# dannyfa/VAE-GAM

Hardware: AMD Instinct MI355X
Metric: fMRI volumes/sec/train-step (41x49x35) (higher is better)
Workload: dtype f32; 1 GPU; configs[2] full VAE-GAM: B=64/GPU C=8, 41x49x35, 2 subj x 98 vol synthetic checker, fwd+bwd+Adam, hipGraph replay; global_batch=64, covariates=8, parallelism=dp1

## Files before the change

include/vaegam.h:

```cpp
#ifndef VAEGAM_H
#define VAEGAM_H
#include <stdint.h>
#ifdef __cplusplus
extern "C" {
#endif

typedef struct vg_conv_desc {
    int32_t N;
    int32_t CI, CO;
    int32_t ID, IH, IW;
    int32_t OD, OH, OW;
    int32_t KD, KH, KW;
    int32_t stride;
    int32_t pad_d, pad_h, pad_w;
    int32_t relu_in;
    int32_t per_group;
    int32_t relu_out;
} vg_conv_desc;

int         vg_version(void);
const char* vg_last_error(void);

int vg_corr3d(const vg_conv_desc* d, const float* x, const float* wpk, const float* bias,
              const float* in_scale, const float* in_shift, const float* mask_src, float* y, void* stream);

int vg_tconv3d_s2(const vg_conv_desc* d, const float* x, const float* wpk, const float* bias,
                  const float* in_scale, const float* in_shift, const float* mask_src, float* y, void* stream);
int64_t vg_tconv3d_s2_stats_chunks(const vg_conv_desc* d, int32_t stats_per_group);
int vg_tconv3d_s2_stats(const vg_conv_desc* d, const float* x, const float* wpk, const float* bias,
                        const float* in_scale, const float* in_shift, float* y, int32_t stats_per_group,
                        int32_t stats_relu, double* stats_part, void* stream);

#define VG_CONV_PLAN_LEN 36
int vg_corr3d_plan(const vg_conv_desc* d, int32_t has_prologue, int32_t* out, int32_t n_out);
int vg_tconv3d_s2_plan(const vg_conv_desc* d, int32_t has_prologue, int32_t stats_per_group, int32_t* out, int32_t n_out);

typedef struct vg_mm_desc {
    int32_t N, CI, CO;
    int32_t ID, IH, IW, OD, OH, OW;
    int32_t nq, ks[4];
    int32_t PDT, PH, PW, PD;
    int32_t sdi, shi, swi, d0, LD, cc;
    int32_t sdo, sho, swo, od0[4], oh0[4], ow0[4];
    int32_t relu_in, per_group, tpc, slack;
    int32_t dbuf;
    int32_t PHB;
    int32_t hlo, hhi;
    int32_t waves;
    int32_t relu_out;
} vg_mm_desc;
int64_t vg_conv_mm_stats_chunks(const vg_mm_desc* d, int32_t stats_per_group);
int vg_conv_mm(const vg_mm_desc* d, const float* x, const float* a_img, const int32_t* tau, const int32_t* dlt, const float* bias,
               const float* in_scale, const float* in_shift, const float* mask_src, float* y, int32_t stats_per_group,
               int32_t stats_relu, double* stats_part, void* stream);
int vg_gather_f32(const float* src, const int32_t* idx, float* dst, int64_t n, void* stream);

typedef struct vg_wgrad_desc {
    int32_t N, CB, CA;
    int32_t PD, PH, PW;
    int32_t AD, AH, AW;
    int32_t KD, KH, KW;
    int32_t stride;
    int32_t pad_d, pad_h, pad_w;
    int32_t pro_on_a;
// ... 179 lines not shown
```

vae-gam_amd/_lib.py:

```python
import ctypes
import os

import torch

_HERE = os.path.dirname(os.path.abspath(__file__))
LIB_NAME = 'libvaegam_hip.so'

i32, i64, f32, f64, vp = ctypes.c_int32, ctypes.c_int64, ctypes.c_float, ctypes.c_double, ctypes.c_void_p


class ConvDesc(ctypes.Structure):
    _fields_ = [(n, i32) for n in ('N', 'CI', 'CO', 'ID', 'IH', 'IW', 'OD', 'OH', 'OW', 'KD', 'KH', 'KW',
                                   'stride', 'pad_d', 'pad_h', 'pad_w', 'relu_in', 'per_group', 'relu_out')]


class WgradDesc(ctypes.Structure):
    _fields_ = [(n, i32) for n in ('N', 'CB', 'CA', 'PD', 'PH', 'PW', 'AD', 'AH', 'AW', 'KD', 'KH', 'KW',
                                   'stride', 'pad_d', 'pad_h', 'pad_w', 'pro_on_a', 'relu_in', 'per_group')]


class MmDesc(ctypes.Structure):
    _fields_ = [(n, i32) for n in ('N', 'CI', 'CO', 'ID', 'IH', 'IW', 'OD', 'OH', 'OW', 'nq')] + [('ks', i32 * 4)] + \
               [(n, i32) for n in ('PDT', 'PH', 'PW', 'PD', 'sdi', 'shi', 'swi', 'd0', 'LD', 'cc', 'sdo', 'sho', 'swo')] + \
               [('od0', i32 * 4), ('oh0', i32 * 4), ('ow0', i32 * 4)] + [(n, i32) for n in ('relu_in', 'per_group', 'tpc', 'slack', 'dbuf', 'PHB', 'hlo', 'hhi', 'waves',
                                                                                         'relu_out')]


class GainDesc(ctypes.Structure):
    _fields_ = [('C', i32), ('B', i32), ('n', i32), ('hrf_taps', i32), ('jitter_b', f64), ('jitter_ku', f64), ('prior_var', f64)]


class FcDesc(ctypes.Structure):
    _fields_ = [('M', i32), ('N', i32), ('K', i32), ('batch', i32), ('a_sm', i64), ('a_sk', i64), ('a_sb', i64),
                ('b_sk', i64), ('b_sn', i64), ('b_sb', i64), ('c_sm', i64), ('c_sb', i64), ('bias_sb', i64), ('cx_sb', i64),
                ('ksplit', i32), ('flags', i32)]


class FcJob(ctypes.Structure):
    _fields_ = [('d', FcDesc), ('A', vp), ('amask', vp), ('B', vp), ('bias', vp), ('cmask', vp), ('C', vp), ('cx', vp), ('ws', vp)]

# ... 1 lines not shown
class VolFile(ctypes.Structure):
    _fields_ = [('offset', i64), ('sx', i64), ('sy', i64), ('sz', i64), ('st', i64), ('slope', f64), ('inter', f64),
                ('dtype', i32), ('swap', i32), ('scale', i32), ('reserved', i32)]


FC_A_RELU, FC_A_MASK, FC_B_RELU, FC_B_ONES, FC_C_BIAS, FC_C_RELU, FC_C_MASK, FC_C_ACCUM = 1, 2, 4, 8, 16, 32, 64, 128


_PROTOS = {
    'vg_version': (ctypes.c_int, []),
    'vg_last_error': (ctypes.c_char_p, []),
    'vg_corr3d': (ctypes.c_int, [ctypes.POINTER(ConvDesc), vp, vp, vp, vp, vp, vp, vp, vp]),
    'vg_tconv3d_s2': (ctypes.c_int, [ctypes.POINTER(ConvDesc), vp, vp, vp, vp, vp, vp, vp, vp]),
    'vg_tconv3d_s2_stats_chunks': (i64, [ctypes.POINTER(ConvDesc), i32]),
    'vg_tconv3d_s2_stats': (ctypes.c_int, [ctypes.POINTER(ConvDesc), vp, vp, vp, vp, vp, vp, i32, i32, vp, vp]),
    'vg_corr3d_plan': (ctypes.c_int, [ctypes.POINTER(ConvDesc), i32, ctypes.POINTER(i32), i32]),
    'vg_tconv3d_s2_plan': (ctypes.c_int, [ctypes.POINTER(ConvDesc), i32, i32, ctypes.POINTER(i32), i32]),
    'vg_bn_stats_from_parts': (ctypes.c_int, [vp, i32, i32, i64, f64, vp, vp, f32, vp, vp, vp, vp, vp, vp, vp]),
    'vg_wgrad3d_ws_bytes': (i64, [ctypes.POINTER(WgradDesc)]),
    'vg_wgrad3d': (ctypes.c_int, [ctypes.POINTER(WgradDesc), vp, vp, vp, vp, vp, vp, i32, vp]),
    'vg_wgrad3d_grouped_ws_bytes': (i64, [ctypes.POINTER(WgradDesc)]),
    'vg_wgrad3d_grouped': (ctypes.c_int, [ctypes.POINTER(WgradDesc), vp, vp, vp, vp, vp, vp, vp]),
    'vg_wgrad3d_plan': (ctypes.c_int, [ctypes.POINTER(WgradDesc), i32, ctypes.POINTER(i32), i32]),
    'vg_bn_tconv1_sums': (ctypes.c_int, [vp, vp, vp, vp, i32, i32, i32, vp, vp, i32, vp]),
    'vg_bn_ws_bytes': (i64, [i32, i32, i64, i32]),
    'vg_bn_plan': (ctypes.c_int, [i32, i32, i64, i32, ctypes.POINTER(i32)]),
    'vg_bn_stats': (ctypes.c_int, [vp, i32, i32, i64, i32, i32, vp, vp, f32, vp, vp, vp, vp, vp, vp, vp]),
    'vg_bn_finalize': (ctypes.c_int, [vp, i32, i32, vp, vp, f32, vp, vp, vp, vp, vp]),
    'vg_bn_bwd_reduce': (ctypes.c_int, [vp, vp, i32, i32, i64, i32, i32, vp, vp, vp, vp, vp]),
    'vg_bn_bwd_apply': (ctypes.c_int, [vp, vp, i32, i32, i64, i32, i32, vp, vp, vp, vp, f64, vp, vp, vp, vp, i32, vp]),
# ... 105 lines not shown
```

vae-gam_amd/csrc/vg_conv.hip:

```cpp
#include "vg_common.h"
#include <stdlib.h>
#include "../../include/vaegam.h"

namespace {

struct CorrParams {
    vg_conv_desc d;
    int TWG, TH, TD;
    int tilesW, tilesH, tilesD;
};

__device__ __forceinline__ int clampi(int v, int lo, int hi) { return min(max(v, lo), hi); }

struct ConvQuery { int32_t* plan; int64_t* chunks; int small; };
enum { FAM_DIRECT = 0, FAM_PLANE = 1, FAM_TCONV = 2 };

template <int COT, int KD, int KH, int KW, int S, int TDt, int THt, int TW, int COC>
__global__ void __launch_bounds__(256)
corr3d_direct_k(const float* __restrict__ x, const float* __restrict__ wpk, const float* __restrict__ bias,
         const float* __restrict__ in_scale, const float* __restrict__ in_shift,
         const float* __restrict__ mask_src, float* __restrict__ y, CorrParams p) {
    constexpr int KVOL = KD * KH * KW;
    constexpr int RW = (TW - 1) * S + KW;
    constexpr int RD = (TDt - 1) * S + KD;
// ... 637 lines not shown
        const size_t chunks = (size_t)stats_pg * gridDim.x * nw;
        const size_t chunk = ((size_t)(n % stats_pg) * gridDim.x + blockIdx.x) * nw + wv;
#pragma unroll
        for (int co = 0; co < COT; ++co) {
            float a = st_s[co], b = st_q[co];
#pragma unroll
            for (int off = 32; off > 0; off >>= 1) { a += __shfl_xor(a, off); b += __shfl_xor(b, off); }
            if (lane == 0) {
                double* dst = stats_part + (((size_t)g * CO + co0 + co) * chunks + chunk) * 2;
                dst[0] = (double)a; dst[1] = (double)b;
            }
        }
    }
}

template <int COT, int KD, int KH, int KW, int COC = 0>
int launch_tconv(const vg_conv_desc* d, const float* x, const float* wpk, const float* bias, const float* in_scale,
                 const float* in_shift, const float* mask_src, float* y, hipStream_t s,
                 double* stats_part = nullptr, int stats_relu = 0, int stats_pg = 1, const ConvQuery* query = nullptr) {
    TconvParams p; p.d = *d;
    p.JD = (d->OD + d->pad_d + 1) / 2; p.JH = (d->OH + d->pad_h + 1) / 2; p.JW = (d->OW + d->pad_w + 1) / 2;
    p.TJW = p.JW < 32 ? p.JW : 32;
    int rem = 256 / p.TJW;
    p.TJH = p.JH < rem ? p.JH : rem;
    rem = 256 / (p.TJW * p.TJH);
    p.TJD = p.JD < rem ? p.JD : rem;
    if (p.TJD < 1) p.TJD = 1;
    p.tilesW = vg_cdiv(p.JW, p.TJW); p.tilesH = vg_cdiv(p.JH, p.TJH); p.tilesD = vg_cdiv(p.JD, p.TJD);
    if (d->CO % COT) { vg_set_error("tconv3d_s2: CO=%d not a multiple of %d", d->CO, COT); return VG_ERR_UNSUPPORTED; }
    const int threads = vg_cdiv(p.TJW * p.TJH * p.TJD, VG_WAVE) * VG_WAVE;
    dim3 grid(p.tilesW * p.tilesH * p.tilesD, d->N, d->CO / COT);
    const bool nopro = in_scale == nullptr && !d->relu_in;
    if (query) {
        const int64_t chunks = (int64_t)stats_pg * grid.x * (threads / VG_WAVE);
        if (query->chunks) *query->chunks = chunks;
        if (query->plan) {
            const int32_t rec[VG_CONV_PLAN_LEN] = {
                FAM_TCONV, COT, KD, KH, KW, 2, 2, 2, 2, COC, nopro ? 1 : 0, query->small, p.TJW, p.TJH, p.TJD, p.tilesW, p.tilesH, p.tilesD,
                threads, (int32_t)grid.x, (int32_t)grid.y, (int32_t)grid.z, 0, 0, 0, 0, 0, 0, 0, 0, 0, 0, p.JD, p.JH, p.JW, (int32_t)chunks};
            for (int i = 0; i < VG_CONV_PLAN_LEN; ++i) query->plan[i] = rec[i];
        }
        return VG_OK;
    }
    if (nopro)
        vg_launch(tconv3d_s2_k<COT, KD, KH, KW, COC, true>, grid, dim3(threads), 0, s,
// ... 139 lines not shown
    ConvQuery q = {out, nullptr, 0};
    rc = tconv_dispatch(d, &dummy, &dummy, nullptr, pro, pro, nullptr, &dummy, nullptr, nullptr, 0, stats_per_group > 0 ? stats_per_group : 1, &q);
    if (rc == VG_OK && stats_per_group <= 0) out[VG_CONV_PLAN_LEN - 1] = 0;
    return rc;
}

extern "C" int vg_tconv3d_s2_stats(const vg_conv_desc* d, const float* x, const float* wpk, const float* bias,
                                   const float* in_scale, const float* in_shift, float* y, int32_t stats_per_group,
                                   int32_t stats_relu, double* stats_part, void* stream) {
    int rc = tconv_check(d, x, wpk, in_scale, in_shift, y);
    if (rc) return rc;
    if (!stats_part || stats_per_group <= 0 || d->N % stats_per_group) { vg_set_error("vg_tconv3d_s2_stats: bad statistics arguments"); return VG_ERR_ARG; }
    return tconv_dispatch(d, x, wpk, bias, in_scale, in_shift, nullptr, y, (hipStream_t)stream, stats_part, stats_relu,
                          stats_per_group, nullptr);
}
```

vae-gam_amd/csrc/vg_conv_mm.hip:

```cpp
#include "vg_common.h"
#include <stdlib.h>
#include <stdint.h>
#include <type_traits>
#include "../../include/vaegam.h"

#ifdef VG_STAMP
__device__ unsigned long long vg_stamp_out[1024 * 16 * 8];
#define VG_STAMP_T(t) do { __builtin_amdgcn_sched_barrier(0); asm volatile("s_memtime %0\n\ts_waitcnt lgkmcnt(0)" : "=s"(t) :: "memory"); __builtin_amdgcn_sched_barrier(0); } while (0)
#define VG_STAMP_ADD(i) do { unsigned long long t_; VG_STAMP_T(t_); st_sum[i] += t_ - st_last; st_last = t_; } while (0)
#else
#define VG_STAMP_ADD(i) do {} while (0)
#endif

namespace {

constexpr int MM_MAXQ = 4;
constexpr int MM_ZPAD = 64;

struct MmParams {
    vg_mm_desc d;
    int bps, nsplit;
    int ksbase[MM_MAXQ], a_off[MM_MAXQ];
    int kstot, aimg_floats;
    int a_res;
    int CHP, buf_floats;
    int nhb, PHB, h0, LH, LPH;
    int tau_off, in_off;
    int has_pro;
};

struct alignas(16) mm_f4 { float v[4]; };

template <int V> struct mm_int { static constexpr int value = V; };
template <int MAXN, typename F>
__device__ __forceinline__ void mm_dispatch(int n, F&& f) {
    if constexpr (MAXN >= 1) {
// ... 8 lines not shown

template <int MM_W, int NQ, int TPC, int K0, int K1, int K2, int K3, bool DB, int OCC, bool MASKED>
__global__ void __launch_bounds__(MM_W * VG_WAVE, OCC)
conv_mm_k(const float* __restrict__ x, const float* __restrict__ a_img, const int* __restrict__ tau, const int* __restrict__ dlt,
          const float* __restrict__ bias, const float* __restrict__ in_scale, const float* __restrict__ in_shift,
          const float* __restrict__ mask_src, float* __restrict__ y, double* __restrict__ stats_part, int stats_pg, int stats_relu,
          MmParams p) {
    VG_DYN_SMEM(float, lds);
    constexpr int MM_T = MM_W * VG_WAVE;
    const vg_mm_desc& d = p.d;
    float* Al = lds;
    int* Tl = reinterpret_cast<int*>(lds + p.tau_off);
    float* In = lds + p.in_off;
    const int tid = threadIdx.x, lane = tid % VG_WAVE, wave = vg_wave_id();
    const int kk = lane >> 4, jl = lane & 15;
    const int b = blockIdx.x % p.bps, split = blockIdx.x / p.bps;
    const int IHW = d.IH * d.IW, OHW = d.OH * d.OW;
    const int CI = d.CI, CO = d.CO;
    constexpr bool STATIC_K = K0 > 0;
    constexpr int KSUM = K0 + K1 + K2 + K3;

    for (int i = tid; i < p.aimg_floats; i += MM_T) Al[i] = a_img[i];
    if (!STATIC_K) for (int i = tid; i < p.kstot * 64; i += MM_T) {
        const int* e = dlt + ((i >> 6) * 4 + ((i & 63) >> 4)) * 3;
        Tl[i] = e[0] * p.LPH + e[1] * d.IW + e[2];
    }
    for (int i = tid; i < (DB ? 2 : 1) * d.cc * MM_ZPAD; i += MM_T) In[(i / MM_ZPAD) * p.CHP + (i % MM_ZPAD)] = 0.f;

    const int bd = b / p.nhb, bh = b - bd * p.nhb;
    const int pd0 = bd * d.PD, ph0 = bh * p.PHB;
    const int npd = min(d.PD, d.PDT - pd0), nph = min(p.PHB, d.PH - ph0);
// ... 56 lines not shown
            }
        }
    }
    const float lo = d.relu_in ? 0.f : -__builtin_inff();
    const int nchunks = (CI + d.cc - 1) / d.cc;
    const int nsamp = (d.N - split + p.nsplit - 1) / p.nsplit;
    const int units = nsamp * nchunks;

    vg_f32x4 acc[TPC];
#pragma unroll
    for (int i = 0; i < TPC; ++i) { acc[i].v[0] = 0.f; acc[i].v[1] = 0.f; acc[i].v[2] = 0.f; acc[i].v[3] = 0.f; }
    vg_f2 st_s[2] = {{0.f, 0.f}, {0.f, 0.f}}, st_q[2] = {{0.f, 0.f}, {0.f, 0.f}};
    float mreg[MASKED ? TPC : 1][4];
    vg_f2 bias_l[2];
#pragma unroll
    for (int r = 0; r < 2; ++r) { bias_l[r].x = bias ? bias[co_l + 2 * r] : 0.f; bias_l[r].y = bias ? bias[co_l + 2 * r + 1] : 0.f; }
    int nact = 0;
#pragma unroll
    for (int i = 0; i < TPC; ++i) nact += (i * MM_W + wave < ntiles) ? 1 : 0;

    int nst[NQ];
#pragma unroll
    for (int q = 0; q < NQ; ++q) {
        int c4 = 0;
#pragma unroll
        for (int i = 0; i < TPC; ++i) c4 += (vg_any(((vbits >> (q * TPC + i)) & 1u) != 0) && i < nact) ? 4 : 0;
        nst[q] = c4;
    }

    auto load_mask = [&](int n) __attribute__((always_inline)) {
        const char* mn = reinterpret_cast<const char*>(mask_src + (size_t)n * CO * ovol);
#pragma unroll
        for (int i = 0; i < TPC; ++i) {
            const bool okt = i < nact && ((vbits >> i) & 1u);
            const unsigned off = okt ? ob[i] + 4u * (unsigned)(d.od0[0] * OHW + d.oh0[0] * d.OW + d.ow0[0]) : 0u;
#pragma unroll
            for (int r = 0; r < 4; ++r)
                mreg[i][r] = okt ? *reinterpret_cast<const float*>(mn + (size_t)r * ovol * 4 + off) : 0.f;
        }
    };
    auto store_class_t = [&](int n, int q, auto relu_c, auto stats_c, auto srelu_c) __attribute__((always_inline)) {
        constexpr bool RELU = !MASKED && decltype(relu_c)::value;
        constexpr bool STATS = decltype(stats_c)::value, SRELU = decltype(srelu_c)::value;
        const long long cq4 = 4ll * (d.od0[q] * OHW + d.oh0[q] * d.OW + d.ow0[q]);
        const size_t ovol4 = ovol * 4;
        char* yq = reinterpret_cast<char*>(y + (size_t)n * CO * ovol) + cq4;
        const char* mq = reinterpret_cast<const char*>(mask_src + (size_t)n * CO * ovol) + cq4;
        float* yr[4]; const float* mr[4];
#pragma unroll
        for (int r = 0; r < 4; ++r) { yr[r] = reinterpret_cast<float*>(yq + r * ovol4); mr[r] = reinterpret_cast<const float*>(mq + r * ovol4); }
        vg_touch(vbits);
#pragma unroll
        for (int i = 0; i < TPC; ++i) {
            if ((vbits >> (q * TPC + i)) & 1u) {
                vg_touch(ob[i]);
                const unsigned off = ob[i];
                float mk[4];
                if constexpr (MASKED) {
#pragma unroll
                    for (int r = 0; r < 4; ++r) {
                        if constexpr (NQ == 1) mk[r] = mreg[i][r];
                        else mk[r] = vg_load_sbase(mr[r], off);
// ... 48 lines not shown
            else if (emode == 4) store_class_t(n, q, F{}, T{}, T{});
            else store_class_t(n, q, T{}, T{}, F{});
        }
    };
    auto flush_stats = [&](int n) __attribute__((always_inline)) {
        const int g = n / stats_pg;
        const size_t chunks = (size_t)stats_pg * p.bps * MM_W;
        const size_t chunkid = ((size_t)(n % stats_pg) * p.bps + b) * MM_W + wave;
#pragma unroll
        for (int r = 0; r < 4; ++r) {
            float sa = (r & 1) ? st_s[r >> 1].y : st_s[r >> 1].x, sb = (r & 1) ? st_q[r >> 1].y : st_q[r >> 1].x;
#pragma unroll
            for (int off = 8; off > 0; off >>= 1) { sa += __shfl_xor(sa, off); sb += __shfl_xor(sb, off); }
            if (CO == 8) { sa += __shfl_xor(sa, 32); sb += __shfl_xor(sb, 32); }
            if (jl == 0 && (CO == 16 || kk < 2)) {
                double* dst = stats_part + (((size_t)g * CO + co_l + r) * chunks + chunkid) * 2;
                dst[0] = (double)sa; dst[1] = (double)sb;
            }
        }
#pragma unroll
        for (int r = 0; r < 2; ++r) { st_s[r].x = 0.f; st_s[r].y = 0.f; st_q[r].x = 0.f; st_q[r].y = 0.f; }
    };

    const int nsp = d.cc * nspan_c;
    const int parts = (nsp >= MM_W) ? 1 : (MM_W + nsp - 1) / nsp;
    const int head = dst0 & 3;
    const int n4 = (head + span_fl + 3) >> 2;
    const int n4p = (n4 + parts - 1) / parts;
    auto stage = [&](int u) __attribute__((always_inline)) {
        const int n = split + (u / nchunks) * p.nsplit, c0 = (u % nchunks) * d.cc;
        const int cc = min(d.cc, CI - c0);
// ... 157 lines not shown

}

#ifdef VG_STAMP
extern "C" int vg_stamp_read(unsigned long long* dst, int n) {
    return (int)hipMemcpyFromSymbol(dst, HIP_SYMBOL(vg_stamp_out), sizeof(unsigned long long) * n, 0, hipMemcpyDeviceToHost);
}
#endif

static int mm_plan_params(const vg_mm_desc* d, MmParams* p, size_t* shmem, const char* who) {
    if (!d || d->N <= 0 || d->CI <= 0 || (d->CO != 8 && d->CO != 16) || d->nq < 1 || d->nq > MM_MAXQ || d->PD <= 0 || d->PDT <= 0 ||
        d->PH <= 0 || d->PW <= 0 || d->slack < 0 || d->PH > 1023 || d->PW > 1023 || d->PD > 1023 || d->cc <= 0 || d->LD <= 0 || d->tpc <= 0) {
        vg_set_error("%s: bad descriptor", who); return VG_ERR_ARG;
    }
    p->d = *d;
    int row = 0, af = 0;
    for (int q = 0; q < d->nq; ++q) {
        if (d->ks[q] <= 0 || d->ks[q] > 32) { vg_set_error("%s: k-steps per channel must be 1..32 (class %d: %d)", who, q, d->ks[q]); return VG_ERR_ARG; }
        p->ksbase[q] = row; p->a_off[q] = af;
        row += d->ks[q]; af += d->CI * d->ks[q] * 64;
    }
    p->kstot = row; p->aimg_floats = af;
    if (d->nq > 1 && d->cc < d->CI) { vg_set_error("%s: multi-class plans need all input channels in one chunk", who); return VG_ERR_ARG; }
    const int IHW = d->IH * d->IW;
    const int W = d->waves;
    if (W != 4 && W != 8) { vg_set_error("%s: waves per workgroup must be 4 or 8 (got %d)", who, W); return VG_ERR_ARG; }
    if (d->hhi < d->hlo) { vg_set_error("%s: bad row-offset range [%d, %d]", who, d->hlo, d->hhi); return VG_ERR_ARG; }
    p->PHB = (d->PHB > 0 && d->PHB < d->PH) ? d->PHB : d->PH;
    p->nhb = vg_cdiv(d->PH, p->PHB);
    p->h0 = d->hlo;
// ... 22 lines not shown

extern "C" int vg_conv_mm(const vg_mm_desc* d, const float* x, const float* a_img, const int32_t* tau, const int32_t* dlt,
                          const float* bias, const float* in_scale, const float* in_shift, const float* mask_src, float* y,
                          int32_t stats_per_group, int32_t stats_relu, double* stats_part, void* stream) {
    MmParams p{}; size_t shmem;
    int rc = mm_plan_params(d, &p, &shmem, "vg_conv_mm");
    if (rc) return rc;
    if (!x || !a_img || !tau || !dlt || !y) { vg_set_error("vg_conv_mm: null argument"); return VG_ERR_ARG; }
    if ((in_scale == nullptr) != (in_shift == nullptr) || (in_scale && d->per_group <= 0)) { vg_set_error("vg_conv_mm: in_scale/in_shift/per_group inconsistent"); return VG_ERR_ARG; }
    if (stats_part && (stats_per_group <= 0 || d->N % stats_per_group)) { vg_set_error("vg_conv_mm: bad statistics arguments"); return VG_ERR_ARG; }
    p.has_pro = (d->relu_in || in_scale) ? 1 : 0;
    hipStream_t s = (hipStream_t)stream;
    const int threads = d->waves * VG_WAVE;
    auto launch = [&](auto kernel) {
        const int bpc = vg_blocks_per_cu((const void*)kernel, threads, shmem);
        int ns = (256 * bpc) / p.bps; if (ns < 1) ns = 1; if (ns > d->N) ns = d->N;
        p.nsplit = ns;
        vg_launch(kernel, dim3(p.bps * p.nsplit), dim3(threads), shmem, s, x, a_img, (const int*)tau, (const int*)dlt, bias, in_scale, in_shift,
                  mask_src, y, stats_part, (int)(stats_part ? stats_per_group : 1), (int)stats_relu, p);
    };
    const bool db = d->dbuf != 0, mk = mask_src != nullptr, w4 = d->waves == 4;
#define MM_LAUNCH_W(W, NQ, TPC, K0, K1, K2, K3) { \
        constexpr int OCC_ = (TPC * (K0 + K1 + K2 + K3) + 10 * TPC <= 96 && K0 > 0) ? 4 : 2; \
        if (db) { if (mk) launch(conv_mm_k<W, NQ, TPC, K0, K1, K2, K3, true, OCC_, true>); else launch(conv_mm_k<W, NQ, TPC, K0, K1, K2, K3, true, OCC_, false>); } \
        else    { if (mk) launch(conv_mm_k<W, NQ, TPC, K0, K1, K2, K3, false, OCC_, true>); else launch(conv_mm_k<W, NQ, TPC, K0, K1, K2, K3, false, OCC_, false>); } }
#define MM_LAUNCH(NQ, TPC, K0, K1, K2, K3) { if (w4) MM_LAUNCH_W(4, NQ, TPC, K0, K1, K2, K3) else MM_LAUNCH_W(8, NQ, TPC, K0, K1, K2, K3) }
#define MM_TPC(NQ, K0, K1, K2, K3) \
    { if (d->tpc <= 3) MM_LAUNCH(NQ, 3, K0, K1, K2, K3) else if (d->tpc <= 4) MM_LAUNCH(NQ, 4, K0, K1, K2, K3) else if (d->tpc <= 5) MM_LAUNCH(NQ, 5, K0, K1, K2, K3) \
      else if (d->tpc <= 6) MM_LAUNCH(NQ, 6, K0, K1, K2, K3) else MM_LAUNCH(NQ, 8, K0, K1, K2, K3) }
    const int* k = d->ks;
    if (d->nq == 1 && d->tpc <= 8) {
        if (k[0] == 7) MM_TPC(1, 7, 0, 0, 0)
        else if (k[0] == 9) MM_TPC(1, 9, 0, 0, 0)
// ... 32 lines not shown
```

vae-gam_amd/ops.py:

```python
import ctypes
from collections import namedtuple
from dataclasses import dataclass
from typing import Optional, Tuple

import torch

from . import _lib
from ._lib import ConvDesc, WgradDesc

BN_EPS = 1e-5

PROFILE = None
_LABEL = ['']


class label:
    def __init__(self, name):
        self.name = name

    def __enter__(self):
        self.prev = _LABEL[0]; _LABEL[0] = self.name

    def __exit__(self, *a):
        _LABEL[0] = self.prev
# ... 462 lines not shown
    def forward(ctx, p_in, weight, bias, gamma, beta, spec: ConvSpec, relu_in: bool, per_group: int,
                input_is_data: bool, sync, packed=None, next_bn=None, pre_stats=None, producer_bias=None,
                bias_grad_by_consumer=False, relu_out=False, rectified_in=False):
        p_in = p_in.contiguous()
        has_bn = gamma is not None
        assert not rectified_in or relu_in, 'rectified_in: p_in = relu(p) only stands in for p where the layer rectifies its input'
        fwd_relu = relu_in and not (rectified_in and not has_bn)
        assert producer_bias is None or has_bn, 'producer_bias: the hand-off happens in the batch-norm backward'
        scale = shift = mean = rstd = None
        part = None
        with label(spec.name + '/fwd'):
            if has_bn:
                scale, shift, mean, rstd = bn_stats(p_in, gamma, beta, relu_in, per_group, sync, pre_stats)
            mmf = _mm_for(packed, weight, spec, 'fwd', tuple(p_in.shape[2:]), None)
            if mmf is not None:
                y = conv_mm(p_in, mmf[0], mmf[1], bias, fwd_relu, scale, shift, per_group, None, next_bn, relu_out)
            else:
                wf = packed.get(spec.name, 'fwd') if packed is not None else pack_weight(weight, spec, 'fwd')
                y = conv_forward(p_in, wf, bias, spec, fwd_relu, scale, shift, per_group, next_bn, relu_out)
            if next_bn:
                y, part = y
        ctx.spec, ctx.relu_in, ctx.per_group, ctx.input_is_data, ctx.sync, ctx.has_bn = \
            spec, relu_in, per_group, input_is_data, sync, has_bn
        ctx.save_for_backward(p_in, weight, gamma, beta, scale, shift, mean, rstd)
        ctx.bias_ref = bias
        ctx.packed = packed
        ctx.producer_bias, ctx.bias_grad_by_consumer = producer_bias, bool(bias_grad_by_consumer)
        ctx.nout = 2 if next_bn else 1
        if next_bn:
            ctx.mark_non_differentiable(part)
            return y, part
# ... 78 lines not shown
                    dw = dw_t
            else:
                dp = conv_mm(dy, mmb[0], mmb[1], None, False, None, None, 1, None) if mmb is not None else \
                    conv_backward_data(dy, wb, spec, in_size, None)
                dgamma, dbeta = bn_backward_(dp, p_in, gamma, mean, rstd, relu_in, per_group, ctx.sync, beta, pbg)
        else:
            msk = p_in if relu_in else None
            dp = conv_mm(dy, mmb[0], mmb[1], None, False, None, None, 1, msk) if mmb is not None else \
                conv_backward_data(dy, wb, spec, in_size, msk)
        return dp, dw, db, dgamma, dbeta, None, None, None, None, None, None, None


_MM_SKIP = set(filter(None, _os.environ.get('VG_MM_SKIP', '').split(',')))


def mm_wins(plan):
    if plan is None:
        return False
    if _MM_SKIP and 'k%d' % plan.ks[0] in _MM_SKIP and (plan.PDT + plan.PD - 1) // plan.PD > 1:
        return False
    if USE_MM >= 2 or (plan.PDT + plan.PD - 1) // plan.PD == 1:
        return True
    if plan.mode == 'tconv':
        return list(plan.ks) in ([3, 2, 2, 1], [2, 1, 1, 1], [2, 2, 2, 2])
    return plan.ks[0] in (7, 9)


def _mm_for(packed, weight, spec, direction, read_size, write_size):
    if not USE_MM or (direction == 'bwd' and spec.co == 1):
        return None
    if packed is not None:
        got = packed.get_mm(spec.name, direction)
        if got is not None and (got[0].ID, got[0].IH, got[0].IW) == tuple(read_size):
            return got if mm_wins(got[0]) else None
    plan = mm_plan(spec, direction, read_size, write_size)
    if not mm_wins(plan):
# ... 552 lines not shown
          _p(_chk(out)))
    return out


USE_MM =int(_os.environ.get('VG_CONV_MM', '1'))
_MM_LDS_BUDGET = 150 * 1024
_MM_LDS_CU = 160 * 1024
_MM_TUNED = {
    ('corr', 1, 16, 16, (3, 3, 3), (6, 8, 5), (8, 10, 7)): (8, 4, 10, 16, 0),
    ('corr', 1, 16, 16, (3, 3, 3), (8, 10, 7), (6, 8, 5)): (8, 3, 8, 16, 0),
    ('corr', 2, 16, 16, (3, 3, 3), (16, 21, 14), (8, 10, 7)): (8, 2, 10, 8, 0),
    ('corr', 1, 16, 8, (3, 3, 3), (17, 21, 14), (19, 23, 16)): (8, 1, 23, 8, 0),
    ('corr', 1, 8, 16, (3, 3, 3), (19, 23, 16), (17, 21, 14)): (8, 1, 21, 8, 0),
    ('corr', 1, 8, 16, (3, 3, 3), (18, 23, 16), (16, 21, 14)): (8, 2, 11, 8, 1),
    ('tconv', 2, 8, 8, (5, 3, 3), (18, 23, 16), (39, 47, 33)): (8, 2, 12, 8, 1),
}
_MM_WAVES = 8


class MmPlan:

    def __init__(self, **kw):
        self.__dict__.update(kw)
        self._dev = {}

    def tables(self, device):
        key = str(device)
        if key not in self._dev:
            self._dev[key] = (torch.from_numpy(self.tau).to(device), torch.from_numpy(self.dlt).to(device), torch.from_numpy(self.aidx).to(device))
        return self._dev[key]

    def desc(self, N, relu_in, per_group, relu_out=False):
        d = _lib.MmDesc()
        for k in ('CI', 'CO', 'ID', 'IH', 'IW', 'OD', 'OH', 'OW', 'nq', 'PDT', 'PH', 'PW', 'PD', 'sdi', 'shi', 'swi', 'd0', 'LD', 'cc', 'sdo', 'sho',
                  'swo', 'tpc', 'slack', 'dbuf', 'PHB', 'hlo', 'hhi', 'waves'):
            setattr(d, k, int(getattr(self, k)))
        d.N, d.relu_in, d.per_group, d.relu_out = int(N), int(bool(relu_in)), int(per_group), int(bool(relu_out))
        for q in range(4):
            d.ks[q] = int(self.ks[q]) if q < self.nq else 0
            d.od0[q] = int(self.od0[q]) if q < self.nq else 0
            d.oh0[q] = int(self.oh0[q]) if q < self.nq else 0
            d.ow0[q] = int(self.ow0[q]) if q < self.nq else 0
        return d

    def gather(self, weight):
        _, _, aidx = self.tables(weight.device)
        flat = weight.detach().reshape(-1)
        a = flat[aidx.clamp_min(0).long()]
        return torch.where(aidx >= 0, a, torch.zeros_like(a)).contiguous()


def _mm_problem(spec: ConvSpec, direction: str, in_size):
# ... 23 lines not shown
    return 'corr', spec.stride, tuple(spec.pad), spec.co, spec.ci, spec.k, None, (lambda cin, kd, kh, kw, cout: w_at(cout, cin, kd, kh, kw))


_MM_PLANS = {}


def mm_plan(spec: ConvSpec, direction: str, in_size, out_size=None, force=None) -> Optional[MmPlan]:
    import numpy as np
    key = (spec, direction, tuple(in_size), None if out_size is None else tuple(out_size), force)
    if key in _MM_PLANS:
        return _MM_PLANS[key]
    mode, S, pad, CI, CO, K, osz, widx = _mm_problem(spec, direction, tuple(in_size))
    if osz is None:
        osz = tuple(out_size)
    plan = None
    if CO in (8, 16) and CI >= 8 and not (mode == 'tconv' and CO != 8):
        plan = _mm_build(mode, S, pad, CI, CO, K, tuple(in_size), tuple(osz), widx, force)
    _MM_PLANS[key] = plan
    return plan


def _mm_build(mode, S, pad, CI, CO, K, isz, osz, widx, force=None):
    import numpy as np
    KD, KH, KW = K
    ID, IH, IW = isz
    OD, OH, OW = osz
    IHW = IH * IW
    NR = 16 // CO
    classes = []
    if mode == 'corr':
        KWp = KW + (NR - 1) * S
        ent = []
        for kd in range(KD):
            for kh in range(KH):
                for kwp in range(KWp):
                    def tap(rho, kd=kd, kh=kh, kwp=kwp):
                        kw = kwp - rho * S
                        return (kd, kh, kw) if 0 <= kw < KW else None
                    ent.append((kd - pad[0], kh - pad[1], kwp - pad[2], tap))
        classes.append(ent)
        PDT, PH, PW = OD, OH, (OW + NR - 1) // NR
        sdi, shi, swi = S, S, NR * S
        sdo, sho, swo = 1, 1, NR
# ... 17 lines not shown
                classes.append(ent)
                od0.append(rd - pad[0]); oh0.append(rh - pad[1]); ow0.append(-pad[2])
        PDT, PH, PW = (OD + pad[0] + 1) // 2, (OH + pad[1] + 1) // 2, (OW + pad[2] + 1) // 2
        sdi = shi = swi = 1
        sdo = sho = swo = 2
        d0 = -(MDm - 1)
        ld_of = lambda PD: PD + MDm - 1
    nq = len(classes)
    if nq not in (1, 4) or any(len(e) == 0 for e in classes):
        return None
    ks = [(len(e) + 3) // 4 for e in classes]
    if max(ks) > 32:
        return None
    rows = sum(ks)
    tau = np.zeros((rows, 4), np.int32); dlt = np.zeros((rows, 4, 3), np.int32)
    aidx = []
    slack = 0
    r0 = 0
    for q, ent in enumerate(classes):
        a = -np.ones((CI, ks[q], 64), np.int32)
        for s in range(ks[q]):
            for kk in range(4):
                kap = 4 * s + kk
                e = ent[kap] if kap < len(ent) else ent[0]
                dd, dh, dw = e[0], e[1], e[2]
                tau[r0 + s, kk] = dd * IHW + dh * IW + dw
                dlt[r0 + s, kk] = (dd, dh, dw)
                slack = max(slack, abs(dh) * IW + abs(dw) + 1)
                if kap >= len(ent):
                    continue
                for row in range(16):
                    rho, co = row // CO, row % CO
                    t = e[3](rho)
                    if t is None:
                        continue
                    lane = kk * 16 + row
                    for ci in range(CI):
                        a[ci, s, lane] = widx(ci, t[0], t[1], t[2], co)
        aidx.append(a.reshape(-1))
        r0 += ks[q]
    aidx = np.concatenate(aidx)
    tpc_max = (8 if max(ks) <= 12 else 3) if nq == 1 else 4
    hlo, hhi = int(dlt[:, :, 1].min()), int(dlt[:, :, 1].max())
    tuned = _MM_TUNED.get((mode, S, CI, CO, tuple(K), tuple(isz), tuple(osz))) if force is None else None
    pin = force or tuned
    cands = []
    for W in (8, 4):
        for PD in range(min(PDT, 16), 0, -1):
            LD = ld_of(PD)
            for nslab in (1, 2, 3, 4, 6, 8, 12):
                PHB = (PH + nslab - 1) // nslab
                if nslab > 1 and ((PH + PHB - 1) // PHB != nslab or PHB < 2):
                    continue
                npos = PD * PHB * PW
                tpc = (npos + W * 16 - 1) // (W * 16)
                if tpc > tpc_max:
                    continue
                rows_max = min((PHB - 1) * shi + (hhi - hlo) + 1, IH)
                whole = (nslab == 1 and hlo <= 0 and (PH - 1) * shi + hhi + 1 >= IH)
                LPH = IHW if whole else ((rows_max * IW + 3) // 4) * 4 + 4
                CHP = 64 + ((LD * LPH + 63) // 64) * 64
                bps = ((PDT + PD - 1) // PD) * nslab
                for cc in ([CI] if nq > 1 else [c for c in range(CI, 0, -1) if CI % c == 0]):
                    for dbuf in (1, 0):
                        if pin and (W, PD, PHB, cc, dbuf) != tuple(pin):
                            continue
                        lds = (((aidx.size + 63) // 64) * 64 + rows * 64 + (1 + dbuf) * cc * CHP + 64) * 4
                        if lds > _MM_LDS_BUDGET:
                            continue
                        per_simd = 4 if (tpc <= 3 or nq > 1) else 2
                        nblk = min(_MM_LDS_CU // lds, per_simd * 4 // W)
                        if nblk < 1:
                            continue
                        util = npos / float(tpc * W * 16) * (PDT / float(((PDT + PD - 1) // PD) * PD)) * (PH / float(nslab * PHB))
                        halo = ((PD * sdi) / float(LD)) * min(1.0, (PHB * shi) / float(rows_max))
                        wps = nblk * W // 4
                        occ = {1: 0.45, 2: 0.6, 3: 0.8}.get(wps, 1.0)
                        shape = (1.0 if nslab == 1 else 0.85) * (1.0 if W == 8 else 0.9)
                        score = util * (0.5 + 0.5 * halo) * (0.9 + 0.1 * cc / float(CI)) * occ * shape * (1.0 if (dbuf or nblk >= 2) else 0.9)
                        cands.append((score, PD, LD, cc, tpc, dbuf, PHB, W))
    if not cands:
        return None
    _, PD, LD, cc, tpc, dbuf, PHB, W = max(cands, key=lambda c: (round(c[0], 9), c[3], -c[5]))
    tpc = {1: (3 if tpc <= 3 else tpc if tpc <= 6 else 8), 4: 4}[nq]
    return MmPlan(CI=CI, CO=CO, ID=ID, IH=IH, IW=IW, OD=OD, OH=OH, OW=OW, nq=nq, ks=ks, PDT=PDT, PH=PH, PW=PW, PD=PD, sdi=sdi, shi=shi,
                  swi=swi, d0=d0, LD=LD, cc=cc, sdo=sdo, sho=sho, swo=swo, od0=od0, oh0=oh0, ow0=ow0, tpc=tpc, slack=slack, dbuf=dbuf,
                  PHB=PHB, hlo=hlo, hhi=hhi, waves=W,
                  tau=tau.reshape(-1), dlt=dlt.reshape(-1), aidx=aidx, mode=mode)


def conv_mm(x, plan: MmPlan, aimg, bias, relu_in, scale, shift, per_group, mask_src=None, next_bn=None, relu_out=False):
    lib = _lib.get_lib()
    N = x.shape[0]
    assert tuple(x.shape[1:]) == (plan.CI, plan.ID, plan.IH, plan.IW), (tuple(x.shape), plan.CI, plan.ID, plan.IH, plan.IW)
    tau, dlt, _ = plan.tables(x.device)
    d = plan.desc(N, relu_in, per_group if scale is not None else 1, relu_out)
    y = torch.empty((N, plan.CO, plan.OD, plan.OH, plan.OW), dtype=torch.float32, device=x.device)
    _chk(x); _chk(aimg)
    if next_bn:
        chunks = lib.size('vg_conv_mm_stats_chunks', ctypes.byref(d), int(next_bn))
        G = N // int(next_bn)
        part = torch.zeros(G * plan.CO * chunks * 2, dtype=torch.float64, device=x.device)
        _call(x, 'vg_conv_mm', ctypes.byref(d), _p(x), _p(aimg), _p(tau), _p(dlt), _p(bias), _p(scale), _p(shift), _p(mask_src), _p(y),
              int(next_bn), 1, _p(part))
        return y, part
    _call(x, 'vg_conv_mm', ctypes.byref(d), _p(x), _p(aimg), _p(tau), _p(dlt), _p(bias), _p(scale), _p(shift), _p(mask_src), _p(y), 1, 0, None)
    return y
```

Measured before the change: 10330 volumes/s.

## Route CO=16 transposed convs through matrix-core path as two 8-channel halves

Extends the matrix-multiply conv kernel so a 16-output-channel transposed convolution runs as two 8-channel halves in one launch, each half with its own weight image, bias and output offsets. This lets the previously excluded CO=16 tconv layers use the MFMA path instead of the direct tconv kernel. Because the split kernel cannot fuse BN statistics in the matching chunk layout, a separate stats kernel re-reads the output to produce partial sums. It also adds tuned plans for two such layer shapes. The gain from matrix cores is traded against an extra full read of the output and a more complex indexing scheme.

```diff
diff --git a/include/vaegam.h b/include/vaegam.h
--- a/include/vaegam.h
+++ b/include/vaegam.h
@@ -30,6 +30,9 @@
 int vg_tconv3d_s2_stats(const vg_conv_desc* d, const float* x, const float* wpk, const float* bias,
                         const float* in_scale, const float* in_shift, float* y, int32_t stats_per_group,
                         int32_t stats_relu, double* stats_part, void* stream);
+
+int vg_tconv3d_s2_stats_of(const vg_conv_desc* d, const float* y, int32_t stats_per_group, int32_t stats_relu,
+                           double* stats_part, void* stream);
 
 #define VG_CONV_PLAN_LEN 36
 int vg_corr3d_plan(const vg_conv_desc* d, int32_t has_prologue, int32_t* out, int32_t n_out);
@@ -48,6 +51,7 @@
     int32_t hlo, hhi;
     int32_t waves;
     int32_t relu_out;
+    int32_t co_tot;
 } vg_mm_desc;
 int64_t vg_conv_mm_stats_chunks(const vg_mm_desc* d, int32_t stats_per_group);
 int vg_conv_mm(const vg_mm_desc* d, const float* x, const float* a_img, const int32_t* tau, const int32_t* dlt, const float* bias,
diff --git a/vae-gam_amd/_lib.py b/vae-gam_amd/_lib.py
--- a/vae-gam_amd/_lib.py
+++ b/vae-gam_amd/_lib.py
@@ -23,7 +23,7 @@
     _fields_ = [(n, i32) for n in ('N', 'CI', 'CO', 'ID', 'IH', 'IW', 'OD', 'OH', 'OW', 'nq')] + [('ks', i32 * 4)] + \
                [(n, i32) for n in ('PDT', 'PH', 'PW', 'PD', 'sdi', 'shi', 'swi', 'd0', 'LD', 'cc', 'sdo', 'sho', 'swo')] + \
                [('od0', i32 * 4), ('oh0', i32 * 4), ('ow0', i32 * 4)] + [(n, i32) for n in ('relu_in', 'per_group', 'tpc', 'slack', 'dbuf', 'PHB', 'hlo', 'hhi', 'waves',
-                                                                                         'relu_out')]
+                                                                                         'relu_out', 'co_tot')]
 
 
 class GainDesc(ctypes.Structure):
@@ -55,6 +55,7 @@
     'vg_tconv3d_s2': (ctypes.c_int, [ctypes.POINTER(ConvDesc), vp, vp, vp, vp, vp, vp, vp, vp]),
     'vg_tconv3d_s2_stats_chunks': (i64, [ctypes.POINTER(ConvDesc), i32]),
     'vg_tconv3d_s2_stats': (ctypes.c_int, [ctypes.POINTER(ConvDesc), vp, vp, vp, vp, vp, vp, i32, i32, vp, vp]),
+    'vg_tconv3d_s2_stats_of': (ctypes.c_int, [ctypes.POINTER(ConvDesc), vp, i32, i32, vp, vp]),
     'vg_corr3d_plan': (ctypes.c_int, [ctypes.POINTER(ConvDesc), i32, ctypes.POINTER(i32), i32]),
     'vg_tconv3d_s2_plan': (ctypes.c_int, [ctypes.POINTER(ConvDesc), i32, i32, ctypes.POINTER(i32), i32]),
     'vg_bn_stats_from_parts': (ctypes.c_int, [vp, i32, i32, i64, f64, vp, vp, f32, vp, vp, vp, vp, vp, vp, vp]),
diff --git a/vae-gam_amd/csrc/vg_conv.hip b/vae-gam_amd/csrc/vg_conv.hip
--- a/vae-gam_amd/csrc/vg_conv.hip
+++ b/vae-gam_amd/csrc/vg_conv.hip
@@ -675,11 +675,65 @@
     }
 }
 
-template <int COT, int KD, int KH, int KW, int COC = 0>
-int launch_tconv(const vg_conv_desc* d, const float* x, const float* wpk, const float* bias, const float* in_scale,
-                 const float* in_shift, const float* mask_src, float* y, hipStream_t s,
-                 double* stats_part = nullptr, int stats_relu = 0, int stats_pg = 1, const ConvQuery* query = nullptr) {
-    TconvParams p; p.d = *d;
+template <int COT>
+__global__ void __launch_bounds__(256, 4)
+tconv_stats_of_k(const float* __restrict__ y, TconvParams p, double* __restrict__ stats_part, int stats_relu, int stats_pg) {
+    const vg_conv_desc& d = p.d;
+    const int tid = threadIdx.x;
+    const int n = blockIdx.y;
+    int tile = blockIdx.x;
+    const int twi = tile % p.tilesW; tile /= p.tilesW;
+    const int thi = tile % p.tilesH; const int tdi = tile / p.tilesH;
+    const int CO = d.CO;
+    const int co0 = blockIdx.z * COT;
+    const int jwl = tid % p.TJW; const int jhl = (tid / p.TJW) % p.TJH; const int jdl = tid / (p.TJW * p.TJH);
+    const int jd = tdi * p.TJD + jdl, jh = thi * p.TJH + jhl, jw = twi * p.TJW + jwl;
+    const bool active = !(jdl >= p.TJD || jd >= p.JD || jh >= p.JH || jw >= p.JW);
+    const size_t plane = (size_t)d.OH * d.OW;
+    float st_s[COT], st_q[COT];
+#pragma unroll
+    for (int co = 0; co < COT; ++co) { st_s[co] = 0.f; st_q[co] = 0.f; }
+#pragma unroll
+    for (int rd = 0; rd < 2; ++rd) {
+        const int od = 2 * jd + rd - d.pad_d;
+        if (!active || od < 0 || od >= d.OD) continue;
+#pragma unroll
+        for (int rh = 0; rh < 2; ++rh) {
+            const int oh = 2 * jh + rh - d.pad_h;
+            if (oh < 0 || oh >= d.OH) continue;
+#pragma unroll
+            for (int co = 0; co < COT; ++co) {
+                const size_t base = (((size_t)n * CO + co0 + co) * d.OD + od) * plane + (size_t)oh * d.OW;
+                const int ow0 = 2 * jw - d.pad_w;
+#pragma unroll
+                for (int rw = 0; rw < 2; ++rw) {
+                    if (ow0 + rw >= 0 && ow0 + rw < d.OW) {
+                        const float o = y[base + ow0 + rw];
+                        const float h = stats_relu ? vg_max(o, 0.f) : o;
+                        st_s[co] += h; st_q[co] = fmaf(h, h, st_q[co]);
+                    }
+                }
+            }
+        }
+    }
+    const int lane = tid % VG_WAVE, wv = tid / VG_WAVE, nw = blockDim.x / VG_WAVE;
+    const int g = n / stats_pg;
+    const size_t chunks = (size_t)stats_pg * gridDim.x * nw;
+    const size_t chunk = ((size_t)(n % stats_pg) * gridDim.x + blockIdx.x) * nw + wv;
+#pragma unroll
+    for (int co = 0; co < COT; ++co) {
+        float a = st_s[co], b = st_q[co];
+#pragma unroll
+        for (int off = 32; off > 0; off >>= 1) { a += __shfl_xor(a, off); b += __shfl_xor(b, off); }
+        if (lane == 0) {
+            double* dst = stats_part + (((size_t)g * CO + co0 + co) * chunks + chunk) * 2;
+            dst[0] = (double)a; dst[1] = (double)b;
+        }
+    }
+}
+
+static int tconv_geometry(const vg_conv_desc* d, TconvParams* pp) {
+    TconvParams& p = *pp; p.d = *d;
     p.JD = (d->OD + d->pad_d + 1) / 2; p.JH = (d->OH + d->pad_h + 1) / 2; p.JW = (d->OW + d->pad_w + 1) / 2;
     p.TJW = p.JW < 32 ? p.JW : 32;
     int rem = 256 / p.TJW;
@@ -688,8 +742,16 @@
     p.TJD = p.JD < rem ? p.JD : rem;
     if (p.TJD < 1) p.TJD = 1;
     p.tilesW = vg_cdiv(p.JW, p.TJW); p.tilesH = vg_cdiv(p.JH, p.TJH); p.tilesD = vg_cdiv(p.JD, p.TJD);
+    return vg_cdiv(p.TJW * p.TJH * p.TJD, VG_WAVE) * VG_WAVE;
+}
+
+template <int COT, int KD, int KH, int KW, int COC = 0>
+int launch_tconv(const vg_conv_desc* d, const float* x, const float* wpk, const float* bias, const float* in_scale,
+                 const float* in_shift, const float* mask_src, float* y, hipStream_t s,
+                 double* stats_part = nullptr, int stats_relu = 0, int stats_pg = 1, const ConvQuery* query = nullptr) {
+    TconvParams p;
+    const int threads = tconv_geometry(d, &p);
     if (d->CO % COT) { vg_set_error("tconv3d_s2: CO=%d not a multiple of %d", d->CO, COT); return VG_ERR_UNSUPPORTED; }
-    const int threads = vg_cdiv(p.TJW * p.TJH * p.TJD, VG_WAVE) * VG_WAVE;
     dim3 grid(p.tilesW * p.tilesH * p.tilesD, d->N, d->CO / COT);
     const bool nopro = in_scale == nullptr && !d->relu_in;
     if (query) {
@@ -859,3 +921,21 @@
     return tconv_dispatch(d, x, wpk, bias, in_scale, in_shift, nullptr, y, (hipStream_t)stream, stats_part, stats_relu,
                           stats_per_group, nullptr);
 }
+
+extern "C" int vg_tconv3d_s2_stats_of(const vg_conv_desc* d, const float* y, int32_t stats_per_group, int32_t stats_relu,
+                                      double* stats_part, void* stream) {
+    if (!d || !y || !stats_part) { vg_set_error("vg_tconv3d_s2_stats_of: null argument"); return VG_ERR_ARG; }
+    if (d->N <= 0 || d->N > 65535 || d->CO <= 0 || d->OD <= 0 || d->OH <= 0 || d->OW <= 0 || d->pad_d < 0 || d->pad_h < 0 || d->pad_w < 0) {
+        vg_set_error("vg_tconv3d_s2_stats_of: bad shape N=%d CO=%d out=%dx%dx%d", d->N, d->CO, d->OD, d->OH, d->OW); return VG_ERR_ARG;
+    }
+    if (stats_per_group <= 0 || d->N % stats_per_group) { vg_set_error("vg_tconv3d_s2_stats_of: bad statistics arguments"); return VG_ERR_ARG; }
+    if (d->relu_out && !stats_relu) { vg_set_error("vg_tconv3d_s2_stats_of: a rectified tensor does not hold the pre-activation's statistics"); return VG_ERR_ARG; }
+    if (d->CO % 4) { vg_set_error("vg_tconv3d_s2_stats_of: CO=%d not a multiple of 4", d->CO); return VG_ERR_UNSUPPORTED; }
+    TconvParams p;
+    const int threads = tconv_geometry(d, &p);
+    const int cot = d->CO % 8 == 0 ? 8 : 4;
+    dim3 grid(p.tilesW * p.tilesH * p.tilesD, d->N, d->CO / cot);
+    if (cot == 8) vg_launch(tconv_stats_of_k<8>, grid, dim3(threads), 0, (hipStream_t)stream, y, p, stats_part, (int)stats_relu, (int)stats_per_group);
+    else vg_launch(tconv_stats_of_k<4>, grid, dim3(threads), 0, (hipStream_t)stream, y, p, stats_part, (int)stats_relu, (int)stats_per_group);
+    return vg_check_launch("tconv3d_s2_stats_of");
+}
diff --git a/vae-gam_amd/csrc/vg_conv_mm.hip b/vae-gam_amd/csrc/vg_conv_mm.hip
--- a/vae-gam_amd/csrc/vg_conv_mm.hip
+++ b/vae-gam_amd/csrc/vg_conv_mm.hip
@@ -20,6 +20,7 @@
 struct MmParams {
     vg_mm_desc d;
     int bps, nsplit;
+    int nco, cot;
     int ksbase[MM_MAXQ], a_off[MM_MAXQ];
     int kstot, aimg_floats;
     int a_res;
@@ -58,7 +59,9 @@
     float* In = lds + p.in_off;
     const int tid = threadIdx.x, lane = tid % VG_WAVE, wave = vg_wave_id();
     const int kk = lane >> 4, jl = lane & 15;
-    const int b = blockIdx.x % p.bps, split = blockIdx.x / p.bps;
+    const int b = blockIdx.x % p.bps, bq = blockIdx.x / p.bps;
+    const int split = bq / p.nco, half = bq - split * p.nco, co_h = half * d.CO;
+    a_img += (size_t)half * p.aimg_floats;
     const int IHW = d.IH * d.IW, OHW = d.OH * d.OW;
     const int CI = d.CI, CO = d.CO;
     constexpr bool STATIC_K = K0 > 0;
@@ -145,7 +148,7 @@
     float mreg[MASKED ? TPC : 1][4];
     vg_f2 bias_l[2];
 #pragma unroll
-    for (int r = 0; r < 2; ++r) { bias_l[r].x = bias ? bias[co_l + 2 * r] : 0.f; bias_l[r].y = bias ? bias[co_l + 2 * r + 1] : 0.f; }
+    for (int r = 0; r < 2; ++r) { bias_l[r].x = bias ? bias[co_h + co_l + 2 * r] : 0.f; bias_l[r].y = bias ? bias[co_h + co_l + 2 * r + 1] : 0.f; }
     int nact = 0;
 #pragma unroll
     for (int i = 0; i < TPC; ++i) nact += (i * MM_W + wave < ntiles) ? 1 : 0;
@@ -160,7 +163,7 @@
     }
 
     auto load_mask = [&](int n) __attribute__((always_inline)) {
-        const char* mn = reinterpret_cast<const char*>(mask_src + (size_t)n * CO * ovol);
+        const char* mn = reinterpret_cast<const char*>(mask_src + ((size_t)n * p.cot + co_h) * ovol);
 #pragma unroll
         for (int i = 0; i < TPC; ++i) {
             const bool okt = i < nact && ((vbits >> i) & 1u);
@@ -175,8 +178,8 @@
         constexpr bool STATS = decltype(stats_c)::value, SRELU = decltype(srelu_c)::value;
         const long long cq4 = 4ll * (d.od0[q] * OHW + d.oh0[q] * d.OW + d.ow0[q]);
         const size_t ovol4 = ovol * 4;
-        char* yq = reinterpret_cast<char*>(y + (size_t)n * CO * ovol) + cq4;
-        const char* mq = reinterpret_cast<const char*>(mask_src + (size_t)n * CO * ovol) + cq4;
+        char* yq = reinterpret_cast<char*>(y + ((size_t)n * p.cot + co_h) * ovol) + cq4;
+        const char* mq = reinterpret_cast<const char*>(mask_src + ((size_t)n * p.cot + co_h) * ovol) + cq4;
         float* yr[4]; const float* mr[4];
 #pragma unroll
         for (int r = 0; r < 4; ++r) { yr[r] = reinterpret_cast<float*>(yq + r * ovol4); mr[r] = reinterpret_cast<const float*>(mq + r * ovol4); }
@@ -255,7 +258,7 @@
             for (int off = 8; off > 0; off >>= 1) { sa += __shfl_xor(sa, off); sb += __shfl_xor(sb, off); }
             if (CO == 8) { sa += __shfl_xor(sa, 32); sb += __shfl_xor(sb, 32); }
             if (jl == 0 && (CO == 16 || kk < 2)) {
-                double* dst = stats_part + (((size_t)g * CO + co_l + r) * chunks + chunkid) * 2;
+                double* dst = stats_part + (((size_t)g * p.cot + co_h + co_l + r) * chunks + chunkid) * 2;
                 dst[0] = (double)sa; dst[1] = (double)sb;
             }
         }
@@ -443,6 +446,11 @@
         vg_set_error("%s: bad descriptor", who); return VG_ERR_ARG;
     }
     p->d = *d;
+    p->cot = d->co_tot ? d->co_tot : d->CO;
+    p->nco = p->cot / d->CO;
+    if (p->cot <= 0 || p->cot % d->CO || p->nco > 2 || (p->nco == 2 && d->CO != 8)) {
+        vg_set_error("%s: co_tot = %d with CO = %d: a launch covers CO channels, or two halves of 8", who, d->co_tot, d->CO); return VG_ERR_ARG;
+    }
     int row = 0, af = 0;
     for (int q = 0; q < d->nq; ++q) {
         if (d->ks[q] <= 0 || d->ks[q] > 32) { vg_set_error("%s: k-steps per channel must be 1..32 (class %d: %d)", who, q, d->ks[q]); return VG_ERR_ARG; }
@@ -495,9 +503,9 @@
     const int threads = d->waves * VG_WAVE;
     auto launch = [&](auto kernel) {
         const int bpc = vg_blocks_per_cu((const void*)kernel, threads, shmem);
-        int ns = (256 * bpc) / p.bps; if (ns < 1) ns = 1; if (ns > d->N) ns = d->N;
+        int ns = (256 * bpc) / (p.bps * p.nco); if (ns < 1) ns = 1; if (ns > d->N) ns = d->N;
         p.nsplit = ns;
-        vg_launch(kernel, dim3(p.bps * p.nsplit), dim3(threads), shmem, s, x, a_img, (const int*)tau, (const int*)dlt, bias, in_scale, in_shift,
+        vg_launch(kernel, dim3(p.bps * p.nsplit * p.nco), dim3(threads), shmem, s, x, a_img, (const int*)tau, (const int*)dlt, bias, in_scale, in_shift,
                   mask_src, y, stats_part, (int)(stats_part ? stats_per_group : 1), (int)stats_relu, p);
     };
     const bool db = d->dbuf != 0, mk = mask_src != nullptr, w4 = d->waves == 4;
diff --git a/vae-gam_amd/ops.py b/vae-gam_amd/ops.py
--- a/vae-gam_amd/ops.py
+++ b/vae-gam_amd/ops.py
@@ -500,7 +500,8 @@
                 scale, shift, mean, rstd = bn_stats(p_in, gamma, beta, relu_in, per_group, sync, pre_stats)
             mmf = _mm_for(packed, weight, spec, 'fwd', tuple(p_in.shape[2:]), None)
             if mmf is not None:
-                y = conv_mm(p_in, mmf[0], mmf[1], bias, fwd_relu, scale, shift, per_group, None, next_bn, relu_out)
+                y = conv_mm(p_in, mmf[0], mmf[1], bias, fwd_relu, scale, shift, per_group, None, next_bn, relu_out,
+                            stats_like=spec if mmf[0].co_blk != mmf[0].CO else None)
             else:
                 wf = packed.get(spec.name, 'fwd') if packed is not None else pack_weight(weight, spec, 'fwd')
                 y = conv_forward(p_in, wf, bias, spec, fwd_relu, scale, shift, per_group, next_bn, relu_out)
@@ -609,12 +610,21 @@
 _MM_SKIP = set(filter(None, _os.environ.get('VG_MM_SKIP', '').split(',')))
 
 
+def _halves_win(plan):
+    nslab = (plan.PH + plan.PHB - 1) // plan.PHB
+    return ((plan.PDT + plan.PD - 1) // plan.PD) * nslab > 1
+
+
 def mm_wins(plan):
     if plan is None:
         return False
     if _MM_SKIP and 'k%d' % plan.ks[0] in _MM_SKIP and (plan.PDT + plan.PD - 1) // plan.PD > 1:
         return False
-    if USE_MM >= 2 or (plan.PDT + plan.PD - 1) // plan.PD == 1:
+    if USE_MM >= 2:
+        return True
+    if plan.co_blk != plan.CO:
+        return _halves_win(plan)
+    if (plan.PDT + plan.PD - 1) // plan.PD == 1:
         return True
     if plan.mode == 'tconv':
         return list(plan.ks) in ([3, 2, 2, 1], [2, 1, 1, 1], [2, 2, 2, 2])
@@ -1197,6 +1207,8 @@
     ('corr', 1, 8, 16, (3, 3, 3), (19, 23, 16), (17, 21, 14)): (8, 1, 21, 8, 0),
     ('corr', 1, 8, 16, (3, 3, 3), (18, 23, 16), (16, 21, 14)): (8, 2, 11, 8, 1),
     ('tconv', 2, 8, 8, (5, 3, 3), (18, 23, 16), (39, 47, 33)): (8, 2, 12, 8, 1),
+    ('tconv', 2, 16, 16, (3, 3, 3), (8, 10, 7), (16, 21, 14)): (8, 5, 11, 16, 0),
+    ('tconv', 2, 16, 16, (3, 3, 3), (18, 22, 15), (37, 45, 31)): (8, 1, 23, 16, 0),
 }
 _MM_WAVES = 8
 
@@ -1215,10 +1227,11 @@
 
     def desc(self, N, relu_in, per_group, relu_out=False):
         d = _lib.MmDesc()
-        for k in ('CI', 'CO', 'ID', 'IH', 'IW', 'OD', 'OH', 'OW', 'nq', 'PDT', 'PH', 'PW', 'PD', 'sdi', 'shi', 'swi', 'd0', 'LD', 'cc', 'sdo', 'sho',
+        for k in ('CI', 'ID', 'IH', 'IW', 'OD', 'OH', 'OW', 'nq', 'PDT', 'PH', 'PW', 'PD', 'sdi', 'shi', 'swi', 'd0', 'LD', 'cc', 'sdo', 'sho',
                   'swo', 'tpc', 'slack', 'dbuf', 'PHB', 'hlo', 'hhi', 'waves'):
             setattr(d, k, int(getattr(self, k)))
         d.N, d.relu_in, d.per_group, d.relu_out = int(N), int(bool(relu_in)), int(per_group), int(bool(relu_out))
+        d.CO, d.co_tot = int(self.co_blk), int(self.CO)
         for q in range(4):
             d.ks[q] = int(self.ks[q]) if q < self.nq else 0
             d.od0[q] = int(self.od0[q]) if q < self.nq else 0
@@ -1272,7 +1285,7 @@
     if osz is None:
         osz = tuple(out_size)
     plan = None
-    if CO in (8, 16) and CI >= 8 and not (mode == 'tconv' and CO != 8):
+    if CO in (8, 16) and CI >= 8:
         plan = _mm_build(mode, S, pad, CI, CO, K, tuple(in_size), tuple(osz), widx, force)
     _MM_PLANS[key] = plan
     return plan
@@ -1284,7 +1297,9 @@
     ID, IH, IW = isz
     OD, OH, OW = osz
     IHW = IH * IW
-    NR = 16 // CO
+    nco = 2 if (mode == 'tconv' and CO == 16) else 1
+    CO_l = CO // nco
+    NR = 16 // CO_l
     classes = []
     if mode == 'corr':
         KWp = KW + (NR - 1) * S
@@ -1332,11 +1347,11 @@
         return None
     rows = sum(ks)
     tau = np.zeros((rows, 4), np.int32); dlt = np.zeros((rows, 4, 3), np.int32)
-    aidx = []
+    aidx = [[] for _ in range(nco)]
     slack = 0
     r0 = 0
     for q, ent in enumerate(classes):
-        a = -np.ones((CI, ks[q], 64), np.int32)
+        a = -np.ones((nco, CI, ks[q], 64), np.int32)
         for s in range(ks[q]):
             for kk in range(4):
                 kap = 4 * s + kk
@@ -1348,16 +1363,19 @@
                 if kap >= len(ent):
                     continue
                 for row in range(16):
-                    rho, co = row // CO, row % CO
+                    rho, co = row // CO_l, row % CO_l
                     t = e[3](rho)
                     if t is None:
                         continue
                     lane = kk * 16 + row
-                    for ci in range(CI):
-                        a[ci, s, lane] = widx(ci, t[0], t[1], t[2], co)
-        aidx.append(a.reshape(-1))
+                    for h in range(nco):
+                        for ci in range(CI):
+                            a[h, ci, s, lane] = widx(ci, t[0], t[1], t[2], co + CO_l * h)
+        for h in range(nco):
+            aidx[h].append(a[h].reshape(-1))
         r0 += ks[q]
-    aidx = np.concatenate(aidx)
+    aidx = np.concatenate([np.concatenate(a) for a in aidx])
+    aimg_blk = aidx.size // nco
     tpc_max = (8 if max(ks) <= 12 else 3) if nq == 1 else 4
     hlo, hhi = int(dlt[:, :, 1].min()), int(dlt[:, :, 1].max())
     tuned = _MM_TUNED.get((mode, S, CI, CO, tuple(K), tuple(isz), tuple(osz))) if force is None else None
@@ -1383,7 +1401,7 @@
                     for dbuf in (1, 0):
                         if pin and (W, PD, PHB, cc, dbuf) != tuple(pin):
                             continue
-                        lds = (((aidx.size + 63) // 64) * 64 + rows * 64 + (1 + dbuf) * cc * CHP + 64) * 4
+                        lds = (((aimg_blk + 63) // 64) * 64 + rows * 64 + (1 + dbuf) * cc * CHP + 64) * 4
                         if lds > _MM_LDS_BUDGET:
                             continue
                         per_simd = 4 if (tpc <= 3 or nq > 1) else 2
@@ -1401,13 +1419,13 @@
         return None
     _, PD, LD, cc, tpc, dbuf, PHB, W = max(cands, key=lambda c: (round(c[0], 9), c[3], -c[5]))
     tpc = {1: (3 if tpc <= 3 else tpc if tpc <= 6 else 8), 4: 4}[nq]
-    return MmPlan(CI=CI, CO=CO, ID=ID, IH=IH, IW=IW, OD=OD, OH=OH, OW=OW, nq=nq, ks=ks, PDT=PDT, PH=PH, PW=PW, PD=PD, sdi=sdi, shi=shi,
+    return MmPlan(CI=CI, CO=CO, co_blk=CO_l, ID=ID, IH=IH, IW=IW, OD=OD, OH=OH, OW=OW, nq=nq, ks=ks, PDT=PDT, PH=PH, PW=PW, PD=PD, sdi=sdi, shi=shi,
                   swi=swi, d0=d0, LD=LD, cc=cc, sdo=sdo, sho=sho, swo=swo, od0=od0, oh0=oh0, ow0=ow0, tpc=tpc, slack=slack, dbuf=dbuf,
                   PHB=PHB, hlo=hlo, hhi=hhi, waves=W,
                   tau=tau.reshape(-1), dlt=dlt.reshape(-1), aidx=aidx, mode=mode)
 
 
-def conv_mm(x, plan: MmPlan, aimg, bias, relu_in, scale, shift, per_group, mask_src=None, next_bn=None, relu_out=False):
+def conv_mm(x, plan: MmPlan, aimg, bias, relu_in, scale, shift, per_group, mask_src=None, next_bn=None, relu_out=False, stats_like=None):
     lib = _lib.get_lib()
     N = x.shape[0]
     assert tuple(x.shape[1:]) == (plan.CI, plan.ID, plan.IH, plan.IW), (tuple(x.shape), plan.CI, plan.ID, plan.IH, plan.IW)
@@ -1415,6 +1433,14 @@
     d = plan.desc(N, relu_in, per_group if scale is not None else 1, relu_out)
     y = torch.empty((N, plan.CO, plan.OD, plan.OH, plan.OW), dtype=torch.float32, device=x.device)
     _chk(x); _chk(aimg)
+    if next_bn and stats_like is not None:
+        _call(x, 'vg_conv_mm', ctypes.byref(d), _p(x), _p(aimg), _p(tau), _p(dlt), _p(bias), _p(scale), _p(shift), _p(mask_src), _p(y), 1, 0, None)
+        _, cd, osz = conv_fwd_desc(stats_like, N, (plan.ID, plan.IH, plan.IW), relu_in, per_group if scale is not None else 1, relu_out)
+        assert tuple(osz) == (plan.OD, plan.OH, plan.OW) and stats_like.co == plan.CO
+        chunks = lib.size('vg_tconv3d_s2_stats_chunks', ctypes.byref(cd), int(next_bn))
+        part = torch.empty((N // int(next_bn)) * plan.CO * chunks * 2, dtype=torch.float64, device=x.device)
+        _call(x, 'vg_tconv3d_s2_stats_of', ctypes.byref(cd), _p(y), int(next_bn), 1, _p(part))
+        return y, part
     if next_bn:
         chunks = lib.size('vg_conv_mm_stats_chunks', ctypes.byref(d), int(next_bn))
         G = N // int(next_bn)
```

Measured after the change: 10440 volumes/s (median of 6 runs). 1.0% higher.
